# kakaobrain/hqtransformer

Measured on AMD Instinct MI355X. Metric: images/sec (256x256 class-cond sampling), higher is better.
Workload: dtype bf16

## Files before the change

### hqtransformer_amd/csrc/engine.hip

```cpp
#include "../../include/hqt.h"
#include "kernels.h"
#include "fast_kernels.h"
#include "split_kernels.h"
#include "persist.h"

#include <algorithm>
#include <cmath>
#include <cstdarg>
#include <cstdio>
#include <cstring>
#include <map>
#include <memory>
#include <mutex>
#include <string>
#include <vector>

static thread_local std::string g_err;
static int fail(int code, const char* fmt, ...) {
    char buf[1024];
    va_list ap;
    va_start(ap, fmt);
    vsnprintf(buf, sizeof(buf), fmt, ap);
    va_end(ap);
    g_err = buf;
// ... 91 lines not shown
    int max_prefix = 0;
    static constexpr int BODY_BUFS = 10;
    size_t body_bytes[BODY_BUFS] = {};
    int depth_rows = 0;
    int score_chunk = 0;
    int depth_cap() const { return std::max(cfg.max_batch, score_chunk); }
    static constexpr int DEPTH_BUFS = 4;
    size_t depth_bytes[DEPTH_BUFS] = {};
    float *x = nullptr, *xd = nullptr, *logits = nullptr;
    void *hbuf = nullptr, *qbuf = nullptr, *abuf = nullptr, *mbuf = nullptr;
    void *kcache = nullptr, *vcache = nullptr, *dk = nullptr, *dv = nullptr;
    bf16_t *xpk = nullptr, *xdpk = nullptr;
    float *parts = nullptr, *partsd = nullptr;
    int nparts = 0, npartsd = 0;
    float* fold_tmp = nullptr;
    bool tile_gemm = true;
    float* splitk = nullptr;
    size_t splitk_elems = 0;
    struct { const float* slabs; int S; int rows; const float* bias; } pend = {nullptr, 0, 0, nullptr};
    StepState* state = nullptr;
    RowKey* rows = nullptr;
    static constexpr int ROWS_RING = 4;
    RowKey* rows_pinned[ROWS_RING] = {nullptr, nullptr, nullptr, nullptr};
    hipEvent_t rows_ev[ROWS_RING] = {nullptr, nullptr, nullptr, nullptr};
    bool rows_busy[ROWS_RING] = {false, false, false, false};
    int rows_next = 0;
    RowSampler* row_set = nullptr;
    GuidePair* guide = nullptr;
    size_t guide_room() const { return (size_t)std::max(1, cfg.max_batch / 2); }
    unsigned char* keep_mask = nullptr;
// ... 407 lines not shown
        h->Tmax = (c.cond_type == HQT_COND_TEXT ? c.ctx_len_txt : 0) + c.max_steps;
        h->depth_rows = c.code_levels == 3 ? 21 : 5;
        CHK(alloc_body_rows(h.get(), false));
        h->xd = h->logits = nullptr; h->dk = h->dv = nullptr;
        CHK(alloc_depth_ws(h.get(), false));
        const size_t kv = (size_t)c.n_layers * B * h->Tmax * D * 4;
        CHK(dev_alloc(h.get(), &h->kcache, kv, true));
        CHK(dev_alloc(h.get(), &h->vcache, kv, true));
        CHK(dev_alloc(h.get(), (void**)&h->state, sizeof(StepState), true));
        CHK(dev_alloc(h.get(), (void**)&h->rows, B * sizeof(RowKey), true));
        CHK(dev_alloc(h.get(), (void**)&h->row_set, B * sizeof(RowSampler), true));
        CHK(dev_alloc(h.get(), (void**)&h->guide, h->guide_room() * sizeof(GuidePair), true));
        CHK(dev_alloc(h.get(), (void**)&h->keep_mask, B * (size_t)c.max_steps, true));
        CHK(dev_alloc(h.get(), (void**)&h->group_of_row, B * sizeof(int), true));
        CHK(dev_alloc(h.get(), (void**)&h->row_pos, 3 * B * sizeof(int), true));
        CHK(dev_alloc(h.get(), (void**)&h->cond_buf, B * (size_t)std::max(1, c.cond_type == HQT_COND_TEXT ? c.ctx_len_txt : 1) * 8, true));
        CHK(dev_alloc(h.get(), (void**)&h->codes_top, B * (size_t)c.max_steps * 8, true));
        CHK(dev_alloc(h.get(), (void**)&h->codes_bot, B * (size_t)c.max_steps * 4 * 8, true));
        if (c.code_levels == 3) CHK(dev_alloc(h.get(), (void**)&h->codes_l2, B * (size_t)c.max_steps * 16 * 8, true));
        if (!h->parent) {
            CHK(dev_alloc(h.get(), (void**)&h->persist_counters, PERSIST_COUNTER_BYTES, true));
            CHK(dev_alloc(h.get(), (void**)&h->persist_err, 256, true));
            HIPCHK(hipMemset(h->persist_err, 0, 256));
            CHK(dev_alloc(h.get(), (void**)&h->persist_slabs, persist_slab_floats(256) * 4, true));
        } else {
            h->persist_counters = nullptr; h->persist_err = nullptr; h->persist_slabs = nullptr;
        }
    }
    if (c.has_stage1) {
        std::vector<DecLayer> both(h->dec);
// ... 270 lines not shown
        const int dim = c.s1_resample ? E : E << (2 * (L - 1 - l));
        const std::string name = L == 3 ? "stage1.quantizers." + std::to_string(l) + ".embedding"
                                        : (l == 0 ? "stage1.quantize_t.embedding" : "stage1.quantize_b.embedding");
        const float* e = h->w[name].d;
        CHK(dev_alloc(h, (void**)&h->cb_norm[l], (size_t)c.s1_n_embed * 4, false));
        HIPCHK(launch_row_sumsq(e, DT_F32, h->cb_norm[l], c.s1_n_embed, dim, 0));
    }
    h->has_encoder = true;
    return alloc_encode_workspace(h);
}

static std::string key2(const hqt_handle* h, const char* name);

static int finalize_impl(hqt_handle* h);
static int persist_build(hqt_handle* h);
extern "C" int hqt_finalize_weights(hqt_handle* h) {
    if (!h) return fail(HQT_ERR_INVALID, "null handle");
    if (h->finalized) return HQT_OK;
    DeviceGuard dg(h->device);
    if (!dg.ok) return fail(HQT_ERR_HIP, "hipSetDevice(%d) failed", h->device);
    const size_t owned_before = h->owned.size();
    const int rc = finalize_impl(h);
    if (h->fold_tmp) { hipFree(h->fold_tmp); h->fold_tmp = nullptr; }
    if (rc != HQT_OK) {
        hipDeviceSynchronize();
        for (size_t i = owned_before; i < h->owned.size(); ++i) hipFree(h->owned[i]);
        h->owned.resize(owned_before);
        h->body.clear(); h->depth.clear();
        h->pbody = PersistProg(); h->pfull = PersistProg();
        h->head_top = h->head_bot = h->head_l2 = h->post_quant = h->quant_conv = Lin();
        for (auto& l : h->dec) { l.conv1 = l.conv2 = l.nin = l.q = l.k = l.v = l.proj = Lin(); }
        for (auto& l : h->enc) { l.conv1 = l.conv2 = l.nin = l.q = l.k = l.v = l.proj = Lin(); }
        for (auto& p : h->cb_norm) p = nullptr;
        h->vq_h = h->vq_recon = h->vq_zz = h->vq_err = nullptr; h->vq_z = nullptr; h->vq_best = nullptr;
        h->vq_t = h->vq_q = nullptr; h->up_table = nullptr; h->up_lin = h->down_lin = Lin();
        h->has_encoder = false;
    }
    return rc;
}
static int finalize_impl(hqt_handle* h) {
    const hqt_config& c = h->cfg;
    if (c.has_stage2) {
        HIPCHK(hipMalloc((void**)&h->fold_tmp, (size_t)std::max(4 * c.embed_dim, c.vocab_top) * c.embed_dim * 4));
        h->body.resize(c.n_layers);
        h->depth.resize(c.n_layers_depth);
        for (int i = 0; i < c.n_layers; ++i) { CHK(load_block(h, "stage2.blocks." + std::to_string(i), h->body[i])); h->body[i].body = true; }
        for (int i = 0; i < c.n_layers_depth; ++i) CHK(load_block(h, "stage2.depths." + std::to_string(i), h->depth[i]));
        const float* w;
        const int64_t D = c.embed_dim;
        const bool l3 = c.code_levels == 3;
        CHK(get_w(h, key2(h, "head_top.weight"), {c.vocab_top, D}, &w));
// ... 88 lines not shown
                CHK(load_conv(h, l.name + ".v", l.cin, l.cin, 1, l.v));
                CHK(load_conv(h, l.name + ".proj_out", l.cin, l.cin, 1, l.proj));
            } else {
                CHK(get_w(h, "stage1.decoder.norm_out.weight", {l.cin}, &l.n1_g));
                CHK(get_w(h, "stage1.decoder.norm_out.bias", {l.cin}, &l.n1_b));
                CHK(load_conv(h, "decoder.conv_out", l.cout, l.cin, 3, l.conv1));
            }
        }
    }
    if (c.has_stage1 && h->w.count("stage1.encoder.conv_in.weight") && (c.s1_resample != HQT_RESAMPLE_CONV2 || h->w.count("stage1.down_t.weight")))
        CHK(load_encoder(h));
    HIPCHK(stream_gemm_configure());
    HIPCHK(tile_gemm_configure());
    HIPCHK(mfma_gemm_configure());
    HIPCHK(split_kernels_configure());
    HIPCHK(hipDeviceSynchronize());
    h->finalized = true;
    return HQT_OK;
}

struct Mode {
    bool fast = false;
    bool split = false;
    bool split_ar = false;
    int act_dt() const { return fast ? DT_BF16 : DT_F32; }
    size_t act_sz() const { return fast ? 2 : 4; }
};
static int mode_of(int precision, bool stage1, Mode* md) {
    if (precision == HQT_PRECISION_FAST) md->fast = true;
    else if (precision == HQT_PRECISION_SPLIT && stage1) md->split = true;
// ... 8 lines not shown
    g.zero_page = h->zero_page;
    g.tune = h->policy;
    if (g.alpha == 0.0f) g.alpha = 1.0f;
    if (g.lda == 0) g.lda = l.K;
    if (split_planes) { g.Bw = l.w16h; g.Bw_lo = l.w16l; g.Bw_frag16 = l.wfrag16; g.Bw_up16 = l.wup16; }
}

struct SlotName {
    char s[64];
    SlotName(const char* tag, int rows) {
        static const bool by_rows = getenv("HQT_TIMING_BY_ROWS") != nullptr;
        snprintf(s, sizeof s, by_rows ? "%s@%d" : "%s", tag, rows);
    }
};

static int ar_linear(hqt_handle* h, const Mode& md, GemmArgs g, const Lin& l, int a_dt, int c_dt, hipStream_t st,
                     const char* tag, bool defer_residual = false, int* resid_nparts = nullptr) {
    lin_args(h, g, l, false);
    g.k_quarters = 1;
    const SlotName slot(tag, g.M);
    Timed t(h, slot.s, st);
    if (md.fast) {
        if (resid_nparts) *resid_nparts = g.N / 32;
        if ((g.ln_parts ? l.wpk_ln : l.wpk) && h->tile_gemm && tile_gemm_ok(g, a_dt, c_dt)) {
            const TilePlan tp = tile_gemm_plan(g);
            if (tp.geom >= 0 && (size_t)tp.S * 32 * g.a_packed_mb * g.N <= h->splitk_elems) {
                if (g.ln_parts) g.bias = l.bias_ln;
                HIPCHK(launch_tile_gemm(g, g.ln_parts ? l.wpk_ln : l.wpk, a_dt, c_dt, tp, h->splitk, st));
                if (tp.S > 1) {
                    count_variant(h, "variant:tile_gemm_%dx%d_splitk%d:%s", tp.bm, tp.bn, tp.S, slot.s);
                    t.next(SlotName("gemm_combine", g.M).s);
                    HIPCHK(launch_resid_combine(g, h->splitk, tp.S, st));
                } else count_variant(h, "variant:tile_gemm_%dx%d%s:%s", tp.bm, tp.bn, g.ln_parts ? "_dln" : "", slot.s);
                if (resid_nparts) *resid_nparts = tp.S > 1 ? 1 : g.N / tp.bn;
                return HQT_OK;
            }
        }
        if (g.ln_parts) {
            if (!l.wpk_ln || !stream_gemm_ok(g, a_dt, c_dt)) return fail(HQT_ERR_STATE, "deferred-LayerNorm GEMM without folded weights (%s)", tag);
            g.bias = l.bias_ln;
            HIPCHK(launch_stream_gemm(g, l.wpk_ln, a_dt, c_dt, 1, nullptr, st));
            count_variant(h, "variant:stream_gemm_dln:%s", tag);
            return HQT_OK;
        }
        if (l.wpk && stream_gemm_ok(g, a_dt, c_dt)) {
            int S = (defer_residual && g.store != STORE_RESID) ? stream_gemm_splitk(g) : 1;
            if ((size_t)S * 32 * g.a_packed_mb * g.N > h->splitk_elems) S = 1;
            HIPCHK(launch_stream_gemm(g, l.wpk, a_dt, c_dt, S, h->splitk, st));
            count_variant(h, "variant:stream_gemm:%s", tag);
            if (S > 1) h->pend = {h->splitk, S, 32 * g.a_packed_mb, l.b32};
            return HQT_OK;
// ... 86 lines not shown
static std::string key2(const hqt_handle* h, const char* name) {
    std::string n(name);
    if (h->cfg.code_levels == 3) {
        static const char* const tr[][2] = {
            {"tok_emb_top.weight", "tok_emb_levels.0.weight"}, {"tok_emb_bot.weight", "tok_emb_levels.1.weight"},
            {"tok_emb_top_depth.weight", "tok_emb_depth_levels.0.weight"}, {"pos_emb_depth.weight", "pos_emb_depths.0.weight"},
            {"ln_top.weight", "ln_levels.0.weight"}, {"ln_top.bias", "ln_levels.0.bias"},
            {"ln_bot.weight", "ln_levels.1.weight"}, {"ln_bot.bias", "ln_levels.1.bias"},
            {"head_top.weight", "head_levels.0.weight"}, {"head_bot.weight", "head_levels.1.weight"}};
        for (auto& t : tr) if (n == t[0]) { n = t[1]; break; }
    }
    return "stage2." + n;
}
static const float* W(hqt_handle* h, const char* name) { return h->w[key2(h, name)].d; }


struct PackSrc { const float* w; const float* gamma; };

static void persist_block_shapes(hqt_handle* h, const BlockW& bw, bool single_key, int cache_T, int* k4, std::vector<PersistPhase>& out, std::vector<PackSrc>& src) {
    const int D = h->cfg.embed_dim;
    PersistPhase ph{};
    if (single_key) {
        ph.type = PP_KV1; ph.N = 2 * D; ph.K = D; ph.dln = 1; ph.cache_T = cache_T; ph.kv_row = 0;
        out.push_back(ph); src.push_back({bw.qkv.w32 + (size_t)D * D, bw.ln1_g});
    } else {
        ph.type = PP_QKV; ph.N = 3 * D; ph.K = D; ph.dln = 1; ph.cache_T = cache_T;
        out.push_back(ph); src.push_back({bw.qkv.w32, bw.ln1_g});
        ph = PersistPhase{}; ph.type = PP_ATTN; ph.cache_T = cache_T;
        out.push_back(ph); src.push_back({nullptr, nullptr});
    }
// ... 153 lines not shown
    LNArgs ln{x, g, b, add, y, M, D, in_rpg, in_off, 1e-5f, out_dt, out_pk};
    take_pend(h, ln);
    HIPCHK(launch_layernorm(ln, st));
    return HQT_OK;
}

struct Resid { float* x; bf16_t* xpk; float* parts; int* nparts; };

static bool dln_ok(hqt_handle* h, const SampleCtx& c, const BlockW& bw, int M) {
    static const bool off = getenv("HQT_NO_DLN") != nullptr;
    if (off) return false;
    return c.md.fast && M <= PACKED_MAX_ROWS && bw.qkv.wpk_ln && bw.fc1.wpk_ln && bw.proj.wpk && bw.fc2.wpk && h->cfg.embed_dim % 32 == 0;
}

static int run_block(hqt_handle* h, const SampleCtx& c, const BlockW& bw, const Resid& r, int Tq, void* kc, void* vc, int Tcache,
                     int t_base, const int* t_base_dev, int causal) {
    const int D = h->cfg.embed_dim, M = c.B * Tq, adt = c.md.act_dt();
    const bool dln = r.xpk != nullptr;
    const int pk = (dln || (c.md.fast && M <= PACKED_MAX_ROWS && bw.qkv.wpk && bw.proj.wpk && bw.fc1.wpk && bw.fc2.wpk)) ? packed_mb(M) : 0;
    auto normed = [&](GemmArgs& g, const float* gamma, const float* beta, const Lin& l) -> int {
        g.M = M; g.batch = 1; g.a_packed_mb = pk;
        if (dln) { g.A = r.xpk; g.ln_parts = r.parts; g.ln_nparts = *r.nparts; g.ln_colsum = l.colsum; g.ln_eps = 1e-5f; return HQT_OK; }
        g.A = h->hbuf;
        return run_ln(h, c.st, r.x, gamma, beta, nullptr, h->hbuf, M, D, 1, 0, adt, pk);
    };
    auto residual = [&](const void* A, const Lin& l, const char* tag) -> int {
        GemmArgs g{};
        g.A = A; g.M = M; g.batch = 1; g.a_packed_mb = pk; g.C = r.x; g.ldc = D;
        if (dln) { g.store = STORE_RESID; g.resid_pk = r.xpk; g.resid_parts = r.parts; g.c_packed_mb = pk; }
        else { g.store = STORE_ROWS; g.resid = r.x; }
        return ar_linear(h, c.md, g, l, adt, DT_F32, c.st, tag, true, dln ? r.nparts : nullptr);
// ... 2 lines not shown
    CHK(normed(g, bw.ln1_g, bw.ln1_b, bw.qkv));
    g.C = h->qbuf; g.C2 = kc; g.C3 = vc; g.ldc = D; g.qkv_D = D; g.store = STORE_QKV;
    g.rows_per_group = Tq; g.group_stride = Tcache; g.row_offset = t_base; g.row_offset_dev = t_base_dev;
    const int* const row_pos = t_base_dev ? c.row_pos : nullptr;
    g.row_pos = row_pos;
    if (dln && Tq == 1 && t_base == 0 && !t_base_dev && h->single_key) {
        g.qkv_first = 1; g.qkv_v_pk = reinterpret_cast<bf16_t*>(h->abuf); g.c_packed_mb = pk;
        Lin kv = bw.qkv;
        kv.N = 2 * D;
        kv.wpk_ln = bw.qkv.wpk_ln + (size_t)D * bw.qkv.K;
        kv.bias_ln = bw.qkv.bias_ln + D;
        kv.colsum = bw.qkv.colsum + D;
        g.ln_colsum = kv.colsum;
        CHK(ar_linear(h, c.md, g, kv, adt, adt, c.st, "gemm_qkv"));
    } else {
        CHK(ar_linear(h, c.md, g, bw.qkv, adt, adt, c.st, "gemm_qkv"));
        Timed t(h, "attention", c.st);
        AttnArgs a{h->qbuf, kc, vc, h->abuf, c.B, Tq, h->cfg.n_heads, D / h->cfg.n_heads, Tcache, t_base, t_base_dev, causal, adt, pk, nullptr, row_pos};
        if (h->timing) count_variant(h, "variant:attn_%s:%s", attention_kernel_name(attention_choice(a)), r.x == h->xd ? "depth" : "body");
        HIPCHK(launch_attention(a, c.st));
    }
    CHK(residual(h->abuf, bw.proj, "gemm_proj"));
    g = GemmArgs{};
    CHK(normed(g, bw.ln2_g, bw.ln2_b, bw.fc1));
    g.C = h->mbuf; g.ldc = 4 * D;
    g.store = pk ? STORE_PACKED : STORE_ROWS; g.c_packed_mb = pk;
    g.act = h->cfg.gelu_approx ? ACT_GELU_SIGMOID : ACT_GELU_ERF;
    CHK(ar_linear(h, c.md, g, bw.fc1, adt, adt, c.st, "gemm_fc1"));
    return residual(h->mbuf, bw.fc2, "gemm_fc2");
}

// ... 6 lines not shown
    char* const kc = (char*)(stage ? stage->k : h->kcache);
    char* const vc = (char*)(stage ? stage->v : h->vcache);
    const int* tb_dev = body_tbase_from_state ? &h->state->t_base : nullptr;
    const bool dln_body = Tq_body == 1 && dln_ok(h, c, h->body[0], c.B * Tq_body);
    const bool body_persistable = dln_body && body_tbase_from_state && body_t_base == 0;
    *pfull = body_persistable && dln0 && h->single_key && persist_on(h, c, h->pfull);
    const bool pbody = !*pfull && body_persistable && persist_on(h, c, h->pbody);
    if (*pfull) CHK(run_persist(h, c, h->pfull, h->x, 0, tb_dev, "persist_position"));
    if (pbody) CHK(run_persist(h, c, h->pbody, h->x, 1, tb_dev, "persist_body"));
    const Resid r{h->x, dln_body ? h->xpk : nullptr, h->parts, &h->nparts};
    for (int l = 0; l < (pbody || *pfull ? 0 : cf.n_layers); ++l)
        CHK(run_block(h, c, h->body[l], r, Tq_body, kc + l * kv_layer, vc + l * kv_layer, Tcache, body_t_base, tb_dev, 1));
    return HQT_OK;
}

static int run_depth(hqt_handle* h, const SampleCtx& c, bool dln, int Tq, int tbase) {
    const hqt_config& cf = h->cfg;
    const size_t dkv_layer = (size_t)h->depth_cap() * h->depth_rows * cf.embed_dim * c.md.act_sz();
    const Resid r{h->xd, dln ? h->xdpk : nullptr, h->partsd, &h->npartsd};
    for (int l = 0; l < cf.n_layers_depth; ++l)
        CHK(run_block(h, c, h->depth[l], r, Tq, (char*)h->dk + l * dkv_layer, (char*)h->dv + l * dkv_layer, h->depth_rows, tbase, nullptr, 0));
    return HQT_OK;
}

static int head_pk(const SampleCtx& c, const Lin& head, int M) {
    return (c.md.fast && M <= PACKED_MAX_ROWS && head.wpk) ? packed_mb(M) : 0;
}

static int run_head(hqt_handle* h, const SampleCtx& c, const Lin& head, int lv, int M, bool dln, void* normed, float* out = nullptr) {
    static const char* const ln_names[3][2] = {{"ln_top.weight", "ln_top.bias"}, {"ln_bot.weight", "ln_bot.bias"}, {"ln_levels.2.weight", "ln_levels.2.bias"}};
    const int adt = c.md.act_dt(), pk = head_pk(c, head, M);
    GemmArgs g{};
    if (dln) {
        g.A = h->xdpk; g.ln_parts = h->partsd; g.ln_nparts = h->npartsd; g.ln_colsum = head.colsum; g.ln_eps = 1e-5f;
    } else {
        if (!normed) {
// ... 66 lines not shown
}

static int fold_pending(hqt_handle* h, const SampleCtx& c, int M) {
    if (!h->pend.slabs) return HQT_OK;
    return run_ln(h, c.st, h->x, W(h, "ln_f.weight"), W(h, "ln_f.bias"), nullptr, h->hbuf, M, h->cfg.embed_dim, 1, 0, DT_F32, 0);
}

static int run_depth_head(hqt_handle* h, const SampleCtx& c, float* x, int Tq_body, bool pfull) {
    const hqt_config& cf = h->cfg;
    const int D = cf.embed_dim, B = c.B, V = cf.vocab_top;
    const bool bidir = cf.depth_decoding == HQT_DEPTH_BIDIRECTIONAL, causal_head = cf.depth_decoding == HQT_DEPTH_TOP2MID2BOT;
    const int nsub = causal_head ? h->depth_rows : c.levels;
    static const bool fuse_env = !getenv("HQT_NO_FUSED_EMBED");
    const bool fuse = fuse_env && c.levels == 2 && !bidir;
    void* normed[3] = {nullptr, nullptr, nullptr};
    SamplerSet bidir_set;
    if (bidir) {
        const int M = B * h->depth_rows;
        const bool dln = dln_ok(h, c, h->depth[0], M);
        {
            Timed t(h, "bidir_depth_input", c.st);
            LNArgs ln{x, W(h, "ln_f.weight"), W(h, "ln_f.bias"), W(h, "sos_depth"), h->xd, B, D, Tq_body, Tq_body - 1, 1e-5f, DT_F32, 0,
                      nullptr, 0, 0, nullptr, dln ? h->xdpk : nullptr, dln ? packed_mb(M) : 0, h->partsd};
            ln.fill = W(h, "pos_emb_depth.weight");
            take_pend(h, ln);
            HIPCHK(launch_bidir_depth_input(ln, c.st));
            h->npartsd = 1;
        }
        CHK(run_bidir_tail(h, c, dln, normed));
        bidir_set = {c.lv[0].temperature, c.lv[1].top_k, c.lv[1].top_p};
    }
    for (int sub = 0; sub < nsub; ++sub) {
        const SubStep s = sub_step(cf, sub);
        const int M = B * s.Tq;
        const bool dln = depth_dln(h, c, s), in_pfull = pfull && sub == 0;
        if (!bidir && !in_pfull) {
            CHK(run_depth_input(h, c, x, sub, dln, Tq_body, fuse));
            h->npartsd = 1;
            CHK(run_depth(h, c, dln, s.Tq, s.tbase));
        }
        if (!in_pfull) CHK(run_head(h, c, head_of(h, s.lv), s.lv, M, dln, normed[s.lv]));
        if (c.guide) {
            Timed t(h, "guide_logits", c.st);
            HIPCHK(launch_guide_logits(h->logits, h->guide, c.n_guide, V, s.Tq, s.lv, c.st));
        }
        {
            Timed t(h, bidir ? (s.lv ? "bidir_sampler_bot" : "bidir_sampler_top") : "sampler", c.st);
            const SamplerSet& set = bidir ? bidir_set : c.lv[s.lv];
            SamplerArgs sa{h->logits, M, V, s.Tq, B, set.temperature, set.top_k, set.top_p, c.noise, s.tbase,
                           h->state, h->rows, c.n_steps, c.out[s.lv], c.logits_out, h->depth_rows};
            sa.out_stride = s.out_stride; sa.out_slot = s.out_slot;
            sa.fast_math = c.md.fast ? 1 : 0;
            if (c.row_set) {
                sa.row_set = h->row_set; sa.row_top_p = c.row_top_p ? 1 : 0;
                sa.row_lv_t = bidir ? 0 : s.lv; sa.row_lv_k = bidir ? 1 : s.lv;
            }
            if (c.keep) sa.keep = h->keep_mask;
            sa.row_pos = c.row_pos;
            if (fuse && sub == 0) {
                const bool dln_next = depth_dln(h, c, sub_step(cf, 1));
                sa.emb_tok = W(h, "tok_emb_top_depth.weight"); sa.emb_pos = W(h, "pos_emb_depth.weight");
                sa.emb_feed = c.feed[0] != c.out[0] ? c.feed[0] : nullptr;
                sa.emb_x = h->xd; sa.emb_D = D;
                sa.emb_xpk = dln_next ? h->xdpk : nullptr; sa.emb_pk_mb = dln_next ? packed_mb(4 * B) : 0; sa.emb_parts = h->partsd;
            }
            HIPCHK(launch_sampler(sa, c.st));
            const bool report = c.report.any();
            for (int slot = 0; slot < (report || c.logprob_out ? s.Tq : 0); ++slot) {
                t.next(report ? "draw_report" : "code_logprob");
                if (report) HIPCHK(launch_draw_report(sa, c.feed[s.lv], c.logprob_out, c.report, slot, c.st));
                else HIPCHK(launch_code_logprob(sa, c.feed[s.lv], c.logprob_out, slot, c.st));
            }
        }
    }
    return HQT_OK;
}

static int run_position(hqt_handle* h, const SampleCtx& c, int Tq_body, int body_t_base, bool body_tbase_from_state) {
    bool pfull = false;
// ... 722 lines not shown
    CHK(fold_pending(h, cg, n_prompts * T));
    {
        Timed t(h, "prompt_fanout", c.st);
        const FanoutArgs fa{h->pg_k, h->pg_v, h->kcache, h->vcache, h->x, h->pg_x, h->group_of_row, cf.n_layers, c.B, n_prompts, T, D,
                            D * (int)c.md.act_sz(), cf.max_batch, h->Tmax};
        HIPCHK(launch_prompt_fanout(fa, c.st));
    }
    SampleCtx ch = c;
    ch.row_pos = head_row_pos;
    return run_depth_head(h, ch, h->pg_x, 1, false);
}

static std::vector<uint64_t> graph_key_of(const hqt_handle* h, const SampleCtx& c, int G) {
    std::vector<uint64_t> key = {(uint64_t)G, (uint64_t)c.B, (uint64_t)(c.cond != nullptr), (uint64_t)c.noise, (uint64_t)c.logits_out, (uint64_t)c.logprob_out,
                                 (uint64_t)c.precision, (uint64_t)c.n_steps, (uint64_t)c.levels, (uint64_t)h->policy + (c.roll ? 16 : 0),
                                 (uint64_t)((h->persist_enabled && !h->persist_tripped ? 1 : 0) + (h->single_key ? 0 : 4) + (h->split_kslices ? 0 : 8))};
    for (const int64_t* f : c.feed) key.push_back((uint64_t)f);
    for (const SamplerSet& l : c.lv) {
        uint32_t f[2];
        memcpy(f, &l.top_p, 4); memcpy(f + 1, &l.temperature, 4);
        key.push_back((uint64_t)l.top_k); key.push_back(f[0]); key.push_back(f[1]);
    }
    key.push_back((uint64_t)((c.row_set ? 1 : 0) + (c.row_top_p ? 2 : 0)));
    key.push_back((uint64_t)c.n_guide);
    key.push_back(c.keep ? (uint64_t)c.prefix_len + 1 : 0);
    for (const void* p : {(const void*)c.report.entropy, (const void*)c.report.rank, (const void*)c.report.top_codes, (const void*)c.report.top_logprobs}) key.push_back((uint64_t)p);
    key.push_back((uint64_t)c.report.top_n);
    return key;
}
static int capture_steps(hqt_handle* h, const SampleCtx& c, int G) {
    if (h->graph_exec) {
// ... 11 lines not shown
    hipError_t e = hipStreamEndCapture(cc.st, &graph);
    hipStreamDestroy(cc.st);
    if (rc != HQT_OK) { if (graph) hipGraphDestroy(graph); return rc; }
    HIPCHK(e);
    HIPCHK(hipGraphInstantiate(&h->graph_exec, graph, nullptr, nullptr, 0));
    hipGraphDestroy(graph);
    h->graph_has_persist = h->capture_persist;
    h->persist_used = false;
    return HQT_OK;
}

static int sample_run(hqt_handle* h, const SampleCtx& c) {
    const hqt_config& cf = h->cfg;
    HIPCHK(sampler_configure(cf.vocab_top, c.top_p));
    CHK(persist_bind(h));
    if (c.start == 0) HIPCHK(launch_set_step(h->state, 0, 0, c.st));
    if ((c.row_seeds || c.row_offsets) && (!c.row_seeds || !c.row_offsets)) return fail(HQT_ERR_INVALID, "row_seeds and row_offsets come together");
    CHK(send_row_tables(h, c));
    for (int i = 0; i < (c.keep ? c.levels : 0); ++i)
        HIPCHK(launch_copy_kept(c.keep_codes[i], c.out[i], h->keep_mask, c.B, c.n_steps, LEVEL_WIDTH[i], cf.vocab_top, c.st));
    if (!c.row_seeds && !c.guide) HIPCHK(launch_set_rows(h->rows, c.B, c.seed, c.sample_offset, c.st));
    int first = c.start;
    for (int i = 0; i < (c.roll ? c.levels : 0); ++i)
        if (c.feed[i] == c.out[i]) HIPCHK(launch_copy_row_positions(c.roll_prev[i], c.out[i], h->row_pos_received(), c.B, c.n_steps, LEVEL_WIDTH[i], -1, 0, c.st));
    if (c.start > 0) {
    } else if (c.roll) {
        if (c.n_join) CHK(staged_prompt_prefill(h, c, c.n_join, true, h->row_pos_join()));
    } else if (cf.cond_type == HQT_COND_TEXT && c.groups) {
        CHK(staged_prompt_prefill(h, c, c.n_groups, false, nullptr));
        HIPCHK(launch_advance_step(h->state, cf.ctx_len_txt, c.st));
// ... 559 lines not shown
```

### hqtransformer_amd/csrc/kernels.h

```cpp
#pragma once
#include "common.h"

enum { DT_F32 = 0, DT_BF16 = 1 };

hipError_t launch_gemm_generic(const GemmArgs& g, int ta, int tb, int tc, hipStream_t st);
bool exact_mfma_ok(const GemmArgs& g);
hipError_t launch_exact_mfma_gemm(const GemmArgs& g, hipStream_t st);
hipError_t launch_pack_exact_tiles(const float* w, float* out, int N, int K, hipStream_t st);

struct EmbedArgs {
    int B, D, n_steps;
    int embedding;
    int cond_type;
    const StepState* state;
    const int64_t* cond;
    const float* sos;
    const float* tok_top;
    const float* tok_bot;
    const float* pos_top;
    const float* pos_emb;
    const int64_t* codes_top;
    const int64_t* codes_bot;
    float* x;
    bf16_t* xpk;
// ... 115 lines not shown
    const float* emb_pos;
    const int64_t* emb_feed;
    float* emb_x;
    int emb_D;
    bf16_t* emb_xpk;
    int emb_pk_mb;
    float* emb_parts;
    int out_stride, out_slot;
    int fast_math;
    const RowSampler* row_set;
    int row_lv_t, row_lv_k;
    int row_top_p;
    int row_dispatch;
    const unsigned char* keep;
    const int* row_pos;
};
hipError_t launch_sampler(const SamplerArgs& a, hipStream_t st);
hipError_t launch_code_logprob(const SamplerArgs& a, const int64_t* feed, float* logprob, int slot, hipStream_t st);
hipError_t launch_score_logprob(const float* logits, const int64_t* codes, float* logprob, int pairs, int V, int slots, int draw0, int draws, hipStream_t st);
struct ReportOut {
    float* entropy;
    int* rank;
    int top_n;
    int* top_codes;
    float* top_logprobs;
    bool any() const { return entropy || rank || top_n > 0; }
};
hipError_t launch_draw_report(const SamplerArgs& a, const int64_t* feed, float* logprob, const ReportOut& rep, int slot, hipStream_t st);
hipError_t launch_score_report(const float* logits, const int64_t* codes, const ReportOut& rep, int pair0, int pairs, int V, int slots, int draw0, int draws, hipStream_t st);
hipError_t launch_guide_logits(float* logits, const GuidePair* pairs, int n_pairs, int V, int slots, int level, hipStream_t st);
hipError_t launch_depth_embed_l2(const int64_t* codes0, const int64_t* codes1, int n_steps, const StepState* state, const float* tok0,
// ... 102 lines not shown
```

### hqtransformer_amd/csrc/kernels.hip

```cpp
#include "kernels.h"
#include <mutex>
#include "gemm_generic.h"
#include <type_traits>

template <typename T, typename Op>
__device__ __forceinline__ T wave_reduce(T v, Op op) {
#pragma unroll
    for (int off = 32; off > 0; off >>= 1) v = op(v, __shfl_xor(v, off, 64));
    return v;
}
template <typename T, typename Op>
__device__ __forceinline__ T block_reduce(T v, Op op, T* scratch ) {
    v = wave_reduce(v, op);
    const int wid = threadIdx.x >> 6, nw = blockDim.x >> 6;
    __syncthreads();
    if ((threadIdx.x & 63) == 0) scratch[wid] = v;
    __syncthreads();
    T r = scratch[0];
    for (int i = 1; i < nw; ++i) r = op(r, scratch[i]);
    return r;
}
struct OpAdd { template <typename T> __device__ T operator()(T a, T b) const { return a + b; } };
struct OpMax { template <typename T> __device__ T operator()(T a, T b) const { return a > b ? a : b; } };
struct OpMin { template <typename T> __device__ T operator()(T a, T b) const { return a < b ? a : b; } };
// ... 802 lines not shown
        const float ob = __shfl_xor(best, off, 64);
        const int oi = __shfl_xor(besti, off, 64);
        if (ob > best || (ob == best && oi < besti)) { best = ob; besti = oi; }
    }
    __syncthreads();
    if ((tid & 63) == 0) { redf[tid >> 6] = best; redi[tid >> 6] = besti; }
    __syncthreads();
    if (tid == 0) {
        for (int w = 1; w < NT / 64; ++w)
            if (redf[w] > best || (redf[w] == best && redi[w] < besti)) { best = redf[w]; besti = redi[w]; }
        int64_t* const dst = a.out + (a.out_stride > 0 ? ((long long)b * a.n_steps + step) * a.out_stride + a.out_slot : ((long long)b * a.n_steps + step) * a.slots + slot);
        if (idle) {}
        else if (a.keep && a.keep[(long long)b * a.n_steps + step]) besti = (int)*dst;
        else *dst = (int64_t)besti;
        if (a.emb_tok) sel[0] = a.emb_feed ? (int)clamp_idx(a.emb_feed[((long long)b * a.n_steps + step) * a.slots + slot], a.V) : besti;
    }
    if (!a.emb_tok) return;
    __syncthreads();
    const long long code = sel[0];
    const int D = a.emb_D;
#pragma unroll 1
    for (int s4 = 0; s4 < 4; ++s4) {
        const int row = b * 4 + s4;
        float rs = 0.0f, rq = 0.0f;
        for (int d = tid; d < D; d += NT) {
            const float v = a.emb_tok[code * D + d] + a.emb_pos[(long long)s4 * D + d];
            a.emb_x[(long long)row * D + d] = v;
            if (a.emb_xpk) {
                const bf16_t hb = f32_to_bf16(v);
                a.emb_xpk[packed_off(row, d, a.emb_pk_mb)] = hb;
// ... 4 lines not shown
        if (a.emb_xpk) {
#pragma unroll
            for (int off = 32; off > 0; off >>= 1) { rs += __shfl_xor(rs, off, 64); rq += __shfl_xor(rq, off, 64); }
            __syncthreads();
            if ((tid & 63) == 0) { redf[tid >> 6] = rs; dsum[tid >> 6] = (double)rq; }
            __syncthreads();
            if (tid == 0) {
                float ts = 0.0f, tq = 0.0f;
                for (int w = 0; w < NT / 64; ++w) { ts += redf[w]; tq += (float)dsum[w]; }
                a.emb_parts[2 * row] = ts; a.emb_parts[2 * row + 1] = tq;
            }
        }
    }
}

template <int G4>
__global__ __launch_bounds__(256) void sampler_plain_fast_kernel(SamplerArgs a) {
    __shared__ float redf[4];
    __shared__ int redi[4];
    const int V = a.V, tid = threadIdx.x;
    const int r = blockIdx.x, b = r / a.slots, slot = r % a.slots;
    float temperature = a.temperature;
    if (a.row_set) {
        const RowSampler& rs = a.row_set[b];
        temperature = rs.temperature[a.row_lv_t];
        if (!sampler_row_plain(rs.top_k[a.row_lv_k], rs.top_p[a.row_lv_k], V)) return;
    }
    const int step = step_of(a.state, a.row_pos, b);
    const bool idle = row_idle(a.row_pos, b);
    const int draw = a.draw0 + slot;
// ... 50 lines not shown
        const float ob = __shfl_xor(best, off, 64);
        const int oi = __shfl_xor(besti, off, 64);
        if (ob > best || (ob == best && oi < besti)) { best = ob; besti = oi; }
    }
    __syncthreads();
    if ((tid & 63) == 0) { redf[tid >> 6] = best; redi[tid >> 6] = besti; }
    __syncthreads();
    if (tid == 0) {
        for (int w = 1; w < 4; ++w)
            if (redf[w] > best || (redf[w] == best && redi[w] < besti)) { best = redf[w]; besti = redi[w]; }
        int64_t* const dst = a.out + (a.out_stride > 0 ? ((long long)b * a.n_steps + step) * a.out_stride + a.out_slot : ((long long)b * a.n_steps + step) * a.slots + slot);
        if (idle) {}
        else if (a.keep && a.keep[(long long)b * a.n_steps + step]) besti = (int)*dst;
        else *dst = (int64_t)besti;
        if (a.emb_tok) redi[0] = a.emb_feed ? (int)clamp_idx(a.emb_feed[((long long)b * a.n_steps + step) * a.slots + slot], a.V) : besti;
    }
    if (!a.emb_tok) return;
    __shared__ float reds[4][4], redq[4][4];
    __syncthreads();
    const long long code = redi[0];
    const int D = a.emb_D;
    float rs[4] = {0.0f, 0.0f, 0.0f, 0.0f}, rq[4] = {0.0f, 0.0f, 0.0f, 0.0f};
    for (int d = tid; d < D; d += 256) {
        const float t = a.emb_tok[code * D + d];
#pragma unroll
        for (int s4 = 0; s4 < 4; ++s4) {
            const int row = b * 4 + s4;
            const float x = t + a.emb_pos[(long long)s4 * D + d];
            a.emb_x[(long long)row * D + d] = x;
            if (a.emb_xpk) {
                const bf16_t hb = f32_to_bf16(x);
                a.emb_xpk[packed_off(row, d, a.emb_pk_mb)] = hb;
                const float rr = bf16_to_f32(hb);
                rs[s4] += rr; rq[s4] += rr * rr;
            }
        }
    }
    if (a.emb_xpk) {
#pragma unroll
        for (int s4 = 0; s4 < 4; ++s4) {
#pragma unroll
            for (int off = 32; off > 0; off >>= 1) { rs[s4] += __shfl_xor(rs[s4], off, 64); rq[s4] += __shfl_xor(rq[s4], off, 64); }
            if ((tid & 63) == 0) { reds[s4][tid >> 6] = rs[s4]; redq[s4][tid >> 6] = rq[s4]; }
        }
        __syncthreads();
        if (tid < 4) {
            const int row = b * 4 + tid;
            a.emb_parts[2 * row] = ((reds[tid][0] + reds[tid][1]) + reds[tid][2]) + reds[tid][3];
            a.emb_parts[2 * row + 1] = ((redq[tid][0] + redq[tid][1]) + redq[tid][2]) + redq[tid][3];
        }
    }
}

static size_t sampler_smem(int V, bool use_p, int& n2) {
    n2 = 256;
    while (n2 < V) n2 <<= 1;
    size_t sz = 1024 * sizeof(double) + 16 * sizeof(float) + 16 * sizeof(int) + 256 * sizeof(unsigned) + 4 * sizeof(int) +
                (size_t)V * sizeof(float);
    if (use_p) sz += (size_t)n2 * sizeof(float) + (size_t)n2 * sizeof(unsigned short) + (size_t)V;
    return (sz + 15) & ~(size_t)15;
}
hipError_t sampler_configure(int V, bool use_top_p) {
    int n2;
    const size_t smem = sampler_smem(V, use_top_p, n2);
    if (smem > 160 * 1024 || (use_top_p && V > 65536)) return hipErrorInvalidValue;
    static std::mutex mu;
    static size_t limit[64] = {};
    int dev = 0;
    hipError_t e = hipGetDevice(&dev);
    if (e != hipSuccess) return e;
    std::lock_guard<std::mutex> lock(mu);
    if (dev >= 0 && dev < 64 && smem <= limit[dev]) return hipSuccess;
    for (const void* k : {reinterpret_cast<const void*>(sampler_kernel<256, false>), reinterpret_cast<const void*>(sampler_kernel<256, true>),
                          reinterpret_cast<const void*>(sampler_kernel<1024, false>), reinterpret_cast<const void*>(sampler_kernel<1024, true>)}) {
        e = hipFuncSetAttribute(k, hipFuncAttributeMaxDynamicSharedMemorySize, (int)smem);
        if (e != hipSuccess) return e;
    }
    if (e == hipSuccess && dev >= 0 && dev < 64) limit[dev] = smem;
    return e;
}
hipError_t launch_sampler(const SamplerArgs& args, hipStream_t st) {
    SamplerArgs a = args;
    const bool table = a.row_set != nullptr;
    int n2;
    const size_t smem = sampler_smem(a.V, table ? a.row_top_p != 0 : a.top_p > 0.0f, n2);
    if (smem > 160 * 1024) return hipErrorInvalidValue;
    static const bool no_plain = getenv("HQT_NO_PLAIN_SAMPLER") != nullptr;
    const bool plain_v = !no_plain && a.fast_math && a.V % 4 == 0 && a.V <= 8192 && a.V >= 1024;
    a.row_dispatch = table && plain_v ? 1 : 0;
    if (plain_v && (table || sampler_row_plain(a.top_k, a.top_p, a.V))) {
        if (a.V <= 2048) sampler_plain_fast_kernel<2><<<a.R, 256, 0, st>>>(a);
        else if (a.V <= 4096) sampler_plain_fast_kernel<4><<<a.R, 256, 0, st>>>(a);
        else sampler_plain_fast_kernel<8><<<a.R, 256, 0, st>>>(a);
        const hipError_t e = hipGetLastError();
        if (!table || e != hipSuccess) return e;
    }
    if (a.V >= 4096) { if (a.fast_math) sampler_kernel<1024, true><<<a.R, 1024, smem, st>>>(a, n2); else sampler_kernel<1024, false><<<a.R, 1024, smem, st>>>(a, n2); }
    else { if (a.fast_math) sampler_kernel<256, true><<<a.R, 256, smem, st>>>(a, n2); else sampler_kernel<256, false><<<a.R, 256, smem, st>>>(a, n2); }
    return hipGetLastError();
}

template <int G4>
__device__ __forceinline__ float row_max_sel(const float* lg, int code, int V, float4 (&v)[G4], float* sel) {
// ... 897 lines not shown
```

Before: 1702.

## Precompute depth layer-0 QKV table per code and gather instead of GEMM

At finalize time, the first depth block's LayerNorm+QKV projection is precomputed for every (top code, depth position) pair into a bf16 table. During sampling, the sampler records the chosen code, and the depth layer-0 QKV GEMM is replaced by a gather kernel that copies the table rows into q/k/v buffers. This removes a GEMM per depth step at large batch, at the cost of a V*4*3*D bf16 table in memory, extra setup time, and reliance on the depth input being purely a function of the code.

```diff
diff --git a/hqtransformer_amd/csrc/engine.hip b/hqtransformer_amd/csrc/engine.hip
--- a/hqtransformer_amd/csrc/engine.hip
+++ b/hqtransformer_amd/csrc/engine.hip
@@ -129,6 +129,9 @@
     float *parts = nullptr, *partsd = nullptr;
     int nparts = 0, npartsd = 0;
     float* fold_tmp = nullptr;
+    bf16_t* dqt = nullptr;
+    int* dqt_codes = nullptr;
+    bool dqt_on = true;
     bool tile_gemm = true;
     float* splitk = nullptr;
     size_t splitk_elems = 0;
@@ -566,6 +569,7 @@
         CHK(dev_alloc(h.get(), (void**)&h->keep_mask, B * (size_t)c.max_steps, true));
         CHK(dev_alloc(h.get(), (void**)&h->group_of_row, B * sizeof(int), true));
         CHK(dev_alloc(h.get(), (void**)&h->row_pos, 3 * B * sizeof(int), true));
+        CHK(dev_alloc(h.get(), (void**)&h->dqt_codes, B * sizeof(int), true));
         CHK(dev_alloc(h.get(), (void**)&h->cond_buf, B * (size_t)std::max(1, c.cond_type == HQT_COND_TEXT ? c.ctx_len_txt : 1) * 8, true));
         CHK(dev_alloc(h.get(), (void**)&h->codes_top, B * (size_t)c.max_steps * 8, true));
         CHK(dev_alloc(h.get(), (void**)&h->codes_bot, B * (size_t)c.max_steps * 4 * 8, true));
@@ -866,6 +870,7 @@
 
 static int finalize_impl(hqt_handle* h);
 static int persist_build(hqt_handle* h);
+static int build_depth_qkv_table(hqt_handle* h);
 extern "C" int hqt_finalize_weights(hqt_handle* h) {
     if (!h) return fail(HQT_ERR_INVALID, "null handle");
     if (h->finalized) return HQT_OK;
@@ -887,6 +892,7 @@
         h->vq_h = h->vq_recon = h->vq_zz = h->vq_err = nullptr; h->vq_z = nullptr; h->vq_best = nullptr;
         h->vq_t = h->vq_q = nullptr; h->up_table = nullptr; h->up_lin = h->down_lin = Lin();
         h->has_encoder = false;
+        h->dqt = nullptr;
     }
     return rc;
 }
@@ -1005,6 +1011,7 @@
     HIPCHK(tile_gemm_configure());
     HIPCHK(mfma_gemm_configure());
     HIPCHK(split_kernels_configure());
+    if (c.has_stage2) CHK(build_depth_qkv_table(h));
     HIPCHK(hipDeviceSynchronize());
     h->finalized = true;
     return HQT_OK;
@@ -1043,6 +1050,12 @@
     }
 };
 
+static bool tile_path(const hqt_handle* h, const GemmArgs& g, const Lin& l, int a_dt, int c_dt, TilePlan* tp) {
+    if (!(g.ln_parts ? l.wpk_ln : l.wpk) || !h->tile_gemm || !tile_gemm_ok(g, a_dt, c_dt)) return false;
+    *tp = tile_gemm_plan(g);
+    return tp->geom >= 0 && (size_t)tp->S * 32 * g.a_packed_mb * g.N <= h->splitk_elems;
+}
+
 static int ar_linear(hqt_handle* h, const Mode& md, GemmArgs g, const Lin& l, int a_dt, int c_dt, hipStream_t st,
                      const char* tag, bool defer_residual = false, int* resid_nparts = nullptr) {
     lin_args(h, g, l, false);
@@ -1051,19 +1064,17 @@
     Timed t(h, slot.s, st);
     if (md.fast) {
         if (resid_nparts) *resid_nparts = g.N / 32;
-        if ((g.ln_parts ? l.wpk_ln : l.wpk) && h->tile_gemm && tile_gemm_ok(g, a_dt, c_dt)) {
-            const TilePlan tp = tile_gemm_plan(g);
-            if (tp.geom >= 0 && (size_t)tp.S * 32 * g.a_packed_mb * g.N <= h->splitk_elems) {
-                if (g.ln_parts) g.bias = l.bias_ln;
-                HIPCHK(launch_tile_gemm(g, g.ln_parts ? l.wpk_ln : l.wpk, a_dt, c_dt, tp, h->splitk, st));
-                if (tp.S > 1) {
-                    count_variant(h, "variant:tile_gemm_%dx%d_splitk%d:%s", tp.bm, tp.bn, tp.S, slot.s);
-                    t.next(SlotName("gemm_combine", g.M).s);
-                    HIPCHK(launch_resid_combine(g, h->splitk, tp.S, st));
-                } else count_variant(h, "variant:tile_gemm_%dx%d%s:%s", tp.bm, tp.bn, g.ln_parts ? "_dln" : "", slot.s);
-                if (resid_nparts) *resid_nparts = tp.S > 1 ? 1 : g.N / tp.bn;
-                return HQT_OK;
-            }
+        TilePlan tp;
+        if (tile_path(h, g, l, a_dt, c_dt, &tp)) {
+            if (g.ln_parts) g.bias = l.bias_ln;
+            HIPCHK(launch_tile_gemm(g, g.ln_parts ? l.wpk_ln : l.wpk, a_dt, c_dt, tp, h->splitk, st));
+            if (tp.S > 1) {
+                count_variant(h, "variant:tile_gemm_%dx%d_splitk%d:%s", tp.bm, tp.bn, tp.S, slot.s);
+                t.next(SlotName("gemm_combine", g.M).s);
+                HIPCHK(launch_resid_combine(g, h->splitk, tp.S, st));
+            } else count_variant(h, "variant:tile_gemm_%dx%d%s:%s", tp.bm, tp.bn, g.ln_parts ? "_dln" : "", slot.s);
+            if (resid_nparts) *resid_nparts = tp.S > 1 ? 1 : g.N / tp.bn;
+            return HQT_OK;
         }
         if (g.ln_parts) {
             if (!l.wpk_ln || !stream_gemm_ok(g, a_dt, c_dt)) return fail(HQT_ERR_STATE, "deferred-LayerNorm GEMM without folded weights (%s)", tag);
@@ -1180,6 +1191,49 @@
 }
 static const float* W(hqt_handle* h, const char* name) { return h->w[key2(h, name)].d; }
 
+static int build_depth_qkv_table(hqt_handle* h) {
+    const hqt_config& c = h->cfg;
+    h->dqt = nullptr;
+    const char* e = getenv("HQT_DEPTH_QKV_TABLE");
+    if (e && atoi(e) == 0) return HQT_OK;
+    if (c.code_levels != 2 || c.depth_decoding == HQT_DEPTH_BIDIRECTIONAL || c.depth_decoding == HQT_DEPTH_TOP2MID2BOT || !(h->layouts & HQT_LAYOUT_FAST) || c.n_layers_depth < 1) return HQT_OK;
+    const Lin& l = h->depth[0].qkv;
+    const int D = c.embed_dim, V = c.vocab_top;
+    const int CC = std::min(V, 2048), rows = 4 * CC, mb = packed_mb(rows);
+    if (4 * c.max_batch < 512 || rows < 512 || !l.wpk_ln || !l.bias_ln || !l.colsum || l.N != 3 * D) return HQT_OK;
+    GemmArgs g{};
+    g.M = rows; g.batch = 1; g.a_packed_mb = mb; g.ln_nparts = 1; g.ln_colsum = l.colsum; g.ln_eps = 1e-5f;
+    g.ldc = 3 * D; g.qkv_D = D; g.store = STORE_QKV; g.rows_per_group = 1; g.group_stride = 1;
+    lin_args(h, g, l, false);
+    g.k_quarters = 1;
+    g.bias = l.bias_ln;
+    const size_t tbl_bytes = (size_t)V * 4 * 3 * D * sizeof(bf16_t), xpk_bytes = (size_t)mb * 32 * D * sizeof(bf16_t), parts_bytes = (size_t)mb * 32 * 2 * sizeof(float);
+    void *tbl = nullptr, *xpk = nullptr, *parts = nullptr;
+    auto release = [&]() { for (void* p : {tbl, xpk, parts}) if (p) hipFree(p); (void)hipGetLastError(); };
+    if (hipMalloc(&tbl, tbl_bytes) != hipSuccess || hipMalloc(&xpk, xpk_bytes) != hipSuccess || hipMalloc(&parts, parts_bytes) != hipSuccess) { release(); return HQT_OK; }
+    g.A = xpk; g.ln_parts = reinterpret_cast<const float*>(parts);
+    TilePlan tp;
+    if (!tile_path(h, g, l, DT_BF16, DT_BF16, &tp) || tp.S != 1) { release(); return HQT_OK; }
+    const float* tok = W(h, "tok_emb_top_depth.weight");
+    const float* pos = W(h, "pos_emb_depth.weight");
+    hipError_t err = hipMemset(xpk, 0, xpk_bytes);
+    for (int c0 = 0; c0 < V && err == hipSuccess; c0 += CC) {
+        const int code0 = std::min(c0, V - CC);
+        err = launch_depth_table_embed(tok, pos, code0, CC, D, reinterpret_cast<bf16_t*>(xpk), mb, reinterpret_cast<float*>(parts), 0);
+        bf16_t* const out = reinterpret_cast<bf16_t*>(tbl) + (size_t)code0 * 4 * 3 * D;
+        g.C = out; g.C2 = out + D; g.C3 = out + 2 * D;
+        if (err == hipSuccess) err = launch_tile_gemm(g, l.wpk_ln, DT_BF16, DT_BF16, tp, h->splitk, 0);
+    }
+    if (err == hipSuccess) err = hipDeviceSynchronize();
+    hipFree(xpk); hipFree(parts);
+    xpk = parts = nullptr;
+    if (err != hipSuccess) { release(); return fail(HQT_ERR_HIP, "depth q/k/v table: %s", hipGetErrorString(err)); }
+    h->dqt = reinterpret_cast<bf16_t*>(tbl);
+    h->owned.push_back(tbl);
+    h->workspace_bytes += tbl_bytes;
+    return HQT_OK;
+}
+
 
 struct PackSrc { const float* w; const float* gamma; };
 
@@ -1363,7 +1417,7 @@
 }
 
 static int run_block(hqt_handle* h, const SampleCtx& c, const BlockW& bw, const Resid& r, int Tq, void* kc, void* vc, int Tcache,
-                     int t_base, const int* t_base_dev, int causal) {
+                     int t_base, const int* t_base_dev, int causal, const int* qkv_codes = nullptr) {
     const int D = h->cfg.embed_dim, M = c.B * Tq, adt = c.md.act_dt();
     const bool dln = r.xpk != nullptr;
     const int pk = (dln || (c.md.fast && M <= PACKED_MAX_ROWS && bw.qkv.wpk && bw.proj.wpk && bw.fc1.wpk && bw.fc2.wpk)) ? packed_mb(M) : 0;
@@ -1396,7 +1450,18 @@
         g.ln_colsum = kv.colsum;
         CHK(ar_linear(h, c.md, g, kv, adt, adt, c.st, "gemm_qkv"));
     } else {
-        CHK(ar_linear(h, c.md, g, bw.qkv, adt, adt, c.st, "gemm_qkv"));
+        GemmArgs probe = g;
+        lin_args(h, probe, bw.qkv, false);
+        probe.k_quarters = 1;
+        TilePlan tp;
+        if (qkv_codes && dln && c.md.fast && Tq == 4 && tile_path(h, probe, bw.qkv, adt, adt, &tp) && tp.S == 1) {
+            const SlotName slot("depth_qkv_table", M);
+            Timed t(h, slot.s, c.st);
+            const DepthQkvGather ga{h->dqt, qkv_codes, reinterpret_cast<bf16_t*>(g.C), reinterpret_cast<bf16_t*>(g.C2), reinterpret_cast<bf16_t*>(g.C3), c.B, D, h->cfg.vocab_top,
+                                    g.rows_per_group, g.group_stride, g.row_offset, g.row_offset_dev, g.row_pos};
+            HIPCHK(launch_depth_qkv_gather(ga, c.st));
+            count_variant(h, "variant:tile_gemm_table_dln:%s", slot.s);
+        } else CHK(ar_linear(h, c.md, g, bw.qkv, adt, adt, c.st, "gemm_qkv"));
         Timed t(h, "attention", c.st);
         AttnArgs a{h->qbuf, kc, vc, h->abuf, c.B, Tq, h->cfg.n_heads, D / h->cfg.n_heads, Tcache, t_base, t_base_dev, causal, adt, pk, nullptr, row_pos};
         if (h->timing) count_variant(h, "variant:attn_%s:%s", attention_kernel_name(attention_choice(a)), r.x == h->xd ? "depth" : "body");
@@ -1433,12 +1498,12 @@
     return HQT_OK;
 }
 
-static int run_depth(hqt_handle* h, const SampleCtx& c, bool dln, int Tq, int tbase) {
+static int run_depth(hqt_handle* h, const SampleCtx& c, bool dln, int Tq, int tbase, const int* qkv_codes = nullptr) {
     const hqt_config& cf = h->cfg;
     const size_t dkv_layer = (size_t)h->depth_cap() * h->depth_rows * cf.embed_dim * c.md.act_sz();
     const Resid r{h->xd, dln ? h->xdpk : nullptr, h->partsd, &h->npartsd};
     for (int l = 0; l < cf.n_layers_depth; ++l)
-        CHK(run_block(h, c, h->depth[l], r, Tq, (char*)h->dk + l * dkv_layer, (char*)h->dv + l * dkv_layer, h->depth_rows, tbase, nullptr, 0));
+        CHK(run_block(h, c, h->depth[l], r, Tq, (char*)h->dk + l * dkv_layer, (char*)h->dv + l * dkv_layer, h->depth_rows, tbase, nullptr, 0, l == 0 ? qkv_codes : nullptr));
     return HQT_OK;
 }
 
@@ -1535,6 +1600,7 @@
     static const bool fuse_env = !getenv("HQT_NO_FUSED_EMBED");
     const bool fuse = fuse_env && c.levels == 2 && !bidir;
     void* normed[3] = {nullptr, nullptr, nullptr};
+    bool table_codes = false;
     SamplerSet bidir_set;
     if (bidir) {
         const int M = B * h->depth_rows;
@@ -1558,7 +1624,7 @@
         if (!bidir && !in_pfull) {
             CHK(run_depth_input(h, c, x, sub, dln, Tq_body, fuse));
             h->npartsd = 1;
-            CHK(run_depth(h, c, dln, s.Tq, s.tbase));
+            CHK(run_depth(h, c, dln, s.Tq, s.tbase, sub == 1 && table_codes ? h->dqt_codes : nullptr));
         }
         if (!in_pfull) CHK(run_head(h, c, head_of(h, s.lv), s.lv, M, dln, normed[s.lv]));
         if (c.guide) {
@@ -1584,6 +1650,8 @@
                 sa.emb_feed = c.feed[0] != c.out[0] ? c.feed[0] : nullptr;
                 sa.emb_x = h->xd; sa.emb_D = D;
                 sa.emb_xpk = dln_next ? h->xdpk : nullptr; sa.emb_pk_mb = dln_next ? packed_mb(4 * B) : 0; sa.emb_parts = h->partsd;
+                table_codes = h->dqt && h->dqt_on && dln_next && !c.guide && 4 * B >= 512 && sampler_embed_stats_256(sa);
+                if (table_codes) sa.emb_code = h->dqt_codes;
             }
             HIPCHK(launch_sampler(sa, c.st));
             const bool report = c.report.any();
@@ -2336,7 +2404,8 @@
 static std::vector<uint64_t> graph_key_of(const hqt_handle* h, const SampleCtx& c, int G) {
     std::vector<uint64_t> key = {(uint64_t)G, (uint64_t)c.B, (uint64_t)(c.cond != nullptr), (uint64_t)c.noise, (uint64_t)c.logits_out, (uint64_t)c.logprob_out,
                                  (uint64_t)c.precision, (uint64_t)c.n_steps, (uint64_t)c.levels, (uint64_t)h->policy + (c.roll ? 16 : 0),
-                                 (uint64_t)((h->persist_enabled && !h->persist_tripped ? 1 : 0) + (h->single_key ? 0 : 4) + (h->split_kslices ? 0 : 8))};
+                                 (uint64_t)((h->persist_enabled && !h->persist_tripped ? 1 : 0) + (h->single_key ? 0 : 4) + (h->split_kslices ? 0 : 8) +
+                                            (h->dqt && !h->dqt_on ? 32 : 0))};
     for (const int64_t* f : c.feed) key.push_back((uint64_t)f);
     for (const SamplerSet& l : c.lv) {
         uint32_t f[2];
@@ -2378,6 +2447,7 @@
     const hqt_config& cf = h->cfg;
     HIPCHK(sampler_configure(cf.vocab_top, c.top_p));
     CHK(persist_bind(h));
+    { const char* e = getenv("HQT_DEPTH_QKV_TABLE"); h->dqt_on = !(e && atoi(e) == 0); }
     if (c.start == 0) HIPCHK(launch_set_step(h->state, 0, 0, c.st));
     if ((c.row_seeds || c.row_offsets) && (!c.row_seeds || !c.row_offsets)) return fail(HQT_ERR_INVALID, "row_seeds and row_offsets come together");
     CHK(send_row_tables(h, c));
diff --git a/hqtransformer_amd/csrc/kernels.h b/hqtransformer_amd/csrc/kernels.h
--- a/hqtransformer_amd/csrc/kernels.h
+++ b/hqtransformer_amd/csrc/kernels.h
@@ -153,7 +153,20 @@
     int row_dispatch;
     const unsigned char* keep;
     const int* row_pos;
-};
+    int* emb_code;
+};
+bool sampler_embed_stats_256(const SamplerArgs& a);
+hipError_t launch_depth_table_embed(const float* tok, const float* pos, int code0, int codes, int D, bf16_t* xpk, int pk_mb, float* parts, hipStream_t st);
+struct DepthQkvGather {
+    const bf16_t* table;
+    const int* codes;
+    bf16_t *q, *k, *v;
+    int B, D, V;
+    int rows_per_group, group_stride, row_offset;
+    const int* row_offset_dev;
+    const int* row_pos;
+};
+hipError_t launch_depth_qkv_gather(const DepthQkvGather& a, hipStream_t st);
 hipError_t launch_sampler(const SamplerArgs& a, hipStream_t st);
 hipError_t launch_code_logprob(const SamplerArgs& a, const int64_t* feed, float* logprob, int slot, hipStream_t st);
 hipError_t launch_score_logprob(const float* logits, const int64_t* codes, float* logprob, int pairs, int V, int slots, int draw0, int draws, hipStream_t st);
diff --git a/hqtransformer_amd/csrc/kernels.hip b/hqtransformer_amd/csrc/kernels.hip
--- a/hqtransformer_amd/csrc/kernels.hip
+++ b/hqtransformer_amd/csrc/kernels.hip
@@ -840,6 +840,7 @@
         else if (a.keep && a.keep[(long long)b * a.n_steps + step]) besti = (int)*dst;
         else *dst = (int64_t)besti;
         if (a.emb_tok) sel[0] = a.emb_feed ? (int)clamp_idx(a.emb_feed[((long long)b * a.n_steps + step) * a.slots + slot], a.V) : besti;
+        if (a.emb_tok && a.emb_code) a.emb_code[b] = sel[0];
     }
     if (!a.emb_tok) return;
     __syncthreads();
@@ -874,6 +875,71 @@
     }
 }
 
+template <bool WX>
+__device__ __forceinline__ void depth_rows_embed256(const float* __restrict__ tok, const float* __restrict__ pos, float* x, bf16_t* xpk, int pk_mb, float* parts, int b, int D) {
+    __shared__ float reds[4][4], redq[4][4];
+    const int tid = threadIdx.x;
+    float rs[4] = {0.0f, 0.0f, 0.0f, 0.0f}, rq[4] = {0.0f, 0.0f, 0.0f, 0.0f};
+    for (int d = tid; d < D; d += 256) {
+        const float t = tok[d];
+#pragma unroll
+        for (int s4 = 0; s4 < 4; ++s4) {
+            const int row = b * 4 + s4;
+            const float v = t + pos[(long long)s4 * D + d];
+            if (WX) x[(long long)row * D + d] = v;
+            if (xpk) {
+                const bf16_t hb = f32_to_bf16(v);
+                xpk[packed_off(row, d, pk_mb)] = hb;
+                const float rr = bf16_to_f32(hb);
+                rs[s4] += rr; rq[s4] += rr * rr;
+            }
+        }
+    }
+    if (xpk) {
+#pragma unroll
+        for (int s4 = 0; s4 < 4; ++s4) {
+#pragma unroll
+            for (int off = 32; off > 0; off >>= 1) { rs[s4] += __shfl_xor(rs[s4], off, 64); rq[s4] += __shfl_xor(rq[s4], off, 64); }
+            if ((tid & 63) == 0) { reds[s4][tid >> 6] = rs[s4]; redq[s4][tid >> 6] = rq[s4]; }
+        }
+        __syncthreads();
+        if (tid < 4) {
+            const int row = b * 4 + tid;
+            parts[2 * row] = ((reds[tid][0] + reds[tid][1]) + reds[tid][2]) + reds[tid][3];
+            parts[2 * row + 1] = ((redq[tid][0] + redq[tid][1]) + redq[tid][2]) + redq[tid][3];
+        }
+    }
+}
+__global__ __launch_bounds__(256) void depth_table_embed_kernel(const float* tok, const float* pos, int code0, int D, bf16_t* xpk, int pk_mb, float* parts) {
+    depth_rows_embed256<false>(tok + (long long)(code0 + (int)blockIdx.x) * D, pos, nullptr, xpk, pk_mb, parts, blockIdx.x, D);
+}
+hipError_t launch_depth_table_embed(const float* tok, const float* pos, int code0, int codes, int D, bf16_t* xpk, int pk_mb, float* parts, hipStream_t st) {
+    depth_table_embed_kernel<<<codes, 256, 0, st>>>(tok, pos, code0, D, xpk, pk_mb, parts);
+    return hipGetLastError();
+}
+
+__global__ __launch_bounds__(256) void depth_qkv_gather_kernel(DepthQkvGather a) {
+    const int m = blockIdx.x, g = m / a.rows_per_group, D = a.D, n16 = D >> 3;
+    const int b = m >> 2, j = m & 3;
+    const long long code = min(max(a.codes[b], 0), a.V - 1);
+    const uint4* src = reinterpret_cast<const uint4*>(a.table + (code * 4 + j) * 3 * D);
+    const int dev = a.row_offset_dev ? *a.row_offset_dev : 0;
+    const long long row = (long long)g * a.group_stride + m % a.rows_per_group + a.row_offset + (a.row_pos ? row_live(a.row_pos, g) : dev);
+    uint4* const dq = reinterpret_cast<uint4*>(a.q + (long long)m * D);
+    uint4* const dk = reinterpret_cast<uint4*>(a.k + row * D);
+    uint4* const dv = reinterpret_cast<uint4*>(a.v + row * D);
+    for (int i = threadIdx.x; i < 3 * n16; i += 256) {
+        const uint4 val = src[i];
+        const int part = i / n16, c = i - part * n16;
+        (part == 0 ? dq : (part == 1 ? dk : dv))[c] = val;
+    }
+}
+hipError_t launch_depth_qkv_gather(const DepthQkvGather& a, hipStream_t st) {
+    if (a.B <= 0 || a.D % 8 != 0 || a.rows_per_group <= 0) return hipErrorInvalidValue;
+    depth_qkv_gather_kernel<<<4 * a.B, 256, 0, st>>>(a);
+    return hipGetLastError();
+}
+
 template <int G4>
 __global__ __launch_bounds__(256) void sampler_plain_fast_kernel(SamplerArgs a) {
     __shared__ float redf[4];
@@ -954,42 +1020,11 @@
         else if (a.keep && a.keep[(long long)b * a.n_steps + step]) besti = (int)*dst;
         else *dst = (int64_t)besti;
         if (a.emb_tok) redi[0] = a.emb_feed ? (int)clamp_idx(a.emb_feed[((long long)b * a.n_steps + step) * a.slots + slot], a.V) : besti;
+        if (a.emb_tok && a.emb_code) a.emb_code[b] = redi[0];
     }
     if (!a.emb_tok) return;
-    __shared__ float reds[4][4], redq[4][4];
     __syncthreads();
-    const long long code = redi[0];
-    const int D = a.emb_D;
-    float rs[4] = {0.0f, 0.0f, 0.0f, 0.0f}, rq[4] = {0.0f, 0.0f, 0.0f, 0.0f};
-    for (int d = tid; d < D; d += 256) {
-        const float t = a.emb_tok[code * D + d];
-#pragma unroll
-        for (int s4 = 0; s4 < 4; ++s4) {
-            const int row = b * 4 + s4;
-            const float x = t + a.emb_pos[(long long)s4 * D + d];
-            a.emb_x[(long long)row * D + d] = x;
-            if (a.emb_xpk) {
-                const bf16_t hb = f32_to_bf16(x);
-                a.emb_xpk[packed_off(row, d, a.emb_pk_mb)] = hb;
-                const float rr = bf16_to_f32(hb);
-                rs[s4] += rr; rq[s4] += rr * rr;
-            }
-        }
-    }
-    if (a.emb_xpk) {
-#pragma unroll
-        for (int s4 = 0; s4 < 4; ++s4) {
-#pragma unroll
-            for (int off = 32; off > 0; off >>= 1) { rs[s4] += __shfl_xor(rs[s4], off, 64); rq[s4] += __shfl_xor(rq[s4], off, 64); }
-            if ((tid & 63) == 0) { reds[s4][tid >> 6] = rs[s4]; redq[s4][tid >> 6] = rq[s4]; }
-        }
-        __syncthreads();
-        if (tid < 4) {
-            const int row = b * 4 + tid;
-            a.emb_parts[2 * row] = ((reds[tid][0] + reds[tid][1]) + reds[tid][2]) + reds[tid][3];
-            a.emb_parts[2 * row + 1] = ((redq[tid][0] + redq[tid][1]) + redq[tid][2]) + redq[tid][3];
-        }
-    }
+    depth_rows_embed256<true>(a.emb_tok + (long long)redi[0] * a.emb_D, a.emb_pos, a.emb_x, a.emb_xpk, a.emb_pk_mb, a.emb_parts, b, a.emb_D);
 }
 
 static size_t sampler_smem(int V, bool use_p, int& n2) {
@@ -1019,14 +1054,21 @@
     if (e == hipSuccess && dev >= 0 && dev < 64) limit[dev] = smem;
     return e;
 }
+static bool sampler_plain_vocab(const SamplerArgs& a) {
+    static const bool no_plain = getenv("HQT_NO_PLAIN_SAMPLER") != nullptr;
+    return !no_plain && a.fast_math && a.V % 4 == 0 && a.V <= 8192 && a.V >= 1024;
+}
+bool sampler_embed_stats_256(const SamplerArgs& a) {
+    if (a.V < 4096) return true;
+    return sampler_plain_vocab(a) && !a.row_set && sampler_row_plain(a.top_k, a.top_p, a.V);
+}
 hipError_t launch_sampler(const SamplerArgs& args, hipStream_t st) {
     SamplerArgs a = args;
     const bool table = a.row_set != nullptr;
     int n2;
     const size_t smem = sampler_smem(a.V, table ? a.row_top_p != 0 : a.top_p > 0.0f, n2);
     if (smem > 160 * 1024) return hipErrorInvalidValue;
-    static const bool no_plain = getenv("HQT_NO_PLAIN_SAMPLER") != nullptr;
-    const bool plain_v = !no_plain && a.fast_math && a.V % 4 == 0 && a.V <= 8192 && a.V >= 1024;
+    const bool plain_v = sampler_plain_vocab(a);
     a.row_dispatch = table && plain_v ? 1 : 0;
     if (plain_v && (table || sampler_row_plain(a.top_k, a.top_p, a.V))) {
         if (a.V <= 2048) sampler_plain_fast_kernel<2><<<a.R, 256, 0, st>>>(a);
```

Result: no change. 1697 (-0.3%).
